# CompVis/ipoke

Measured on AMD Instinct MI355X. Metric: video-frames/sec (second-stage train step), higher is better.
Workload: dtype bf16; 1 GPU; plants_128 second_stage train, 16x3x128x128 clips, z=64, flow 2048 hidden (1.237 B params), per-GPU batch 20; global_batch=20, clip_frames=16, parallelism=dp1, weights=random init of the named architecture (no checkpoints offline)

## Files before the change

### include/ipoke_hip.h

```cpp
#ifndef IPOKE_HIP_H
#define IPOKE_HIP_H

#include <stdint.h>

#ifdef __cplusplus
extern "C" {
#endif

typedef enum {
  IPOKE_OK = 0,
  IPOKE_ERR_INVALID = -1,
  IPOKE_ERR_HIP = -2,
  IPOKE_ERR_STATE = -3
} ipoke_status;

enum { IPOKE_F32 = 0, IPOKE_BF16 = 1 };
enum { IPOKE_ACT_NONE = 0, IPOKE_ACT_ELU = 1, IPOKE_ACT_RELU = 2, IPOKE_ACT_LRELU02 = 3, IPOKE_ACT_TANH = 4,
       IPOKE_ACT_SIGMOID = 5 };

const char* ipoke_last_error(void);
int ipoke_version(void);
int ipoke_dtype_size(int dtype);

typedef struct {
// ... 22 lines not shown
  int32_t c_scatter;
  int64_t c_sn, c_sh, c_sw, c_row0;
  const float* row_scale;
  int32_t rs_images, rs_stride;
  int32_t w_kmajor;
  int64_t c_sd;
  void* acc_scratch;
  int64_t acc_scratch_bytes;
} ipoke_conv_desc;

int ipoke_conv_forward(const ipoke_conv_desc* d, int dtype, void* stream);
int64_t ipoke_conv_acc_scratch_bytes(int M, int Nout, int splitk);
int ipoke_conv_acc_scratch_init(void* scratch, void* stream);

int ipoke_conv3x3_skinny_splitk(int M, int Kc, int dtype);

typedef struct {
  float* params; float* m; float* v; float* vmax; void* operand;
  float lr, beta1, beta2, eps, weight_decay, grad_scale;
  int32_t step;
  int32_t keep_grad;
} ipoke_wgrad_adam;

typedef struct {
  int32_t NB, Di, Hi, Wi, Do, Ho, Wo, kd, kh, kw, sd, sh, sw, pd, ph, pw, transposed;
  const void* A; int32_t a_f32; int64_t a_sn, a_sd, a_sh, a_sw, a_sc; int32_t a_coff, Kc_real, Kc;
  const void* dY; int32_t ldy; int32_t y_coff; int32_t Nout;
  float* dW; int64_t w_sn, w_sc, w_st;
  int32_t accumulate;
  int32_t splitm;
// ... 377 lines not shown
```

### include/ipoke_hip_dev.h

```cpp
#ifndef IPOKE_HIP_DEV_H
#define IPOKE_HIP_DEV_H

#include "ipoke_hip.h"

#ifdef __cplusplus
extern "C" {
#endif

int ipoke_conv_forward_repeat(const ipoke_conv_desc* d, int dtype, int n, void* stream);
int ipoke_set_dispatch_override(const char* name, int value);
enum { IPOKE_KERNEL_NONE = 0, IPOKE_KERNEL_IGEMM = 1, IPOKE_KERNEL_S8 = 2, IPOKE_KERNEL_HALO = 3, IPOKE_KERNEL_HALO16 = 4, IPOKE_KERNEL_C64 = 5, IPOKE_KERNEL_K8 = 6 };
int ipoke_last_conv_kernel(void);
enum { IPOKE_WGRAD_KERNEL_NONE = 0, IPOKE_WGRAD_KERNEL_TN = 1, IPOKE_WGRAD_KERNEL_TN_GLDS = 2, IPOKE_WGRAD_KERNEL_TN_NARROW = 3,
       IPOKE_WGRAD_KERNEL_LAT8 = 4, IPOKE_WGRAD_KERNEL_HALO = 5 };
int ipoke_last_wgrad_kernel(void);

int ipoke_spin_delay(int us, void* stream);

#define IPOKE_TAG_NT_SQUARE 1
#define IPOKE_TAG_TN_SQUARE 2
#define IPOKE_TAG_UNIT_FWD 3
#define IPOKE_TAG_UNIT_BWD 4
#define IPOKE_TAG_UNIT_INV 5
#define IPOKE_TAG_NN_SQUARE 6
#define IPOKE_TAG_CONV_BASE 16
#define IPOKE_TAG_WGRAD 32
int ipoke_timing_start(void);
int ipoke_timing_start_all(void);
int ipoke_timing_stop(const int* tags, int ntags, int* counts, double* mean_us);
int ipoke_timing_stop_ex(const int* tags, int ntags, int* counts, double* total_us, double* flops, double* bytes);

int ipoke_desc_sizes(int32_t* out, int n);

int ipoke_flow_test_inject_timeout(ipoke_flow* f, int which, void* stream);

int ipoke_gru_set_fused(int mode);

#ifdef __cplusplus
}
#endif
#endif
```

### ipoke_amd/_lib.py

```python
import ctypes
import os
from ctypes import CFUNCTYPE, POINTER, Structure, c_char_p, c_float, c_int, c_int32, c_int64, c_uint32, c_void_p

_HERE = os.path.dirname(os.path.abspath(__file__))
LIB_PATH = os.environ.get("IPOKE_LIB_PATH") or os.path.join(_HERE, "libipoke_hip.so")

F32, BF16 = 0, 1
ACT_NONE, ACT_ELU, ACT_RELU, ACT_LRELU02, ACT_TANH, ACT_SIGMOID = range(6)

DTYPES = {"f32": F32, "fp32": F32, "float32": F32, "bf16": BF16, "bfloat16": BF16}


class ConvDesc(Structure):
    _fields_ = [(n, c_int32) for n in ("NB", "Di", "Hi", "Wi", "Do", "Ho", "Wo", "kd", "kh", "kw", "sd", "sh", "sw",
                                       "pd", "ph", "pw", "transposed")] + [
        ("A", c_void_p), ("a_f32", c_int32),
        ("a_sn", c_int64), ("a_sd", c_int64), ("a_sh", c_int64), ("a_sw", c_int64), ("a_sc", c_int64),
        ("a_coff", c_int32), ("Kc_real", c_int32), ("Kc", c_int32),
        ("W", c_void_p), ("ldw", c_int32), ("Nout", c_int32),
        ("bias", c_void_p), ("act", c_int32), ("dact", c_void_p), ("ld_dact", c_int32), ("dact_act", c_int32),
        ("C", c_void_p), ("c_f32", c_int32), ("c_accumulate", c_int32), ("ldc", c_int64),
        ("c_coff", c_int32), ("c_cstride", c_int32), ("splitk", c_int32),
        ("c_scatter", c_int32), ("c_sn", c_int64), ("c_sh", c_int64), ("c_sw", c_int64), ("c_row0", c_int64),
        ("row_scale", c_void_p), ("rs_images", c_int32), ("rs_stride", c_int32), ("w_kmajor", c_int32), ("c_sd", c_int64),
# ... 104 lines not shown
    "ipoke_conv_forward": (c_int, [POINTER(ConvDesc), c_int, _P]),
    "ipoke_conv_forward_repeat": (c_int, [POINTER(ConvDesc), c_int, c_int, _P]),
    "ipoke_set_dispatch_override": (c_int, [c_char_p, c_int]),
    "ipoke_last_conv_kernel": (c_int, []),
    "ipoke_last_wgrad_kernel": (c_int, []),
    "ipoke_gru_set_fused": (c_int, [c_int]),
    "ipoke_gru_workspace_bytes": (c_int64, [POINTER(GruDesc), c_int]),
    "ipoke_gru_unroll_forward": (c_int, [POINTER(GruDesc), _P, c_int, _P, c_int, POINTER(c_void_p), _P, _P, c_int, c_int, _P]),
    "ipoke_gru_unroll_backward": (c_int, [POINTER(GruDesc), _P, c_int, _P, POINTER(c_void_p), _P, _P, c_int, _P]),
    "ipoke_rowscale_bwd_workspace_floats": (c_int64, [c_int64, c_int, c_int64]),
    "ipoke_rowscale_bwd": (c_int, [POINTER(RowScaleBwdDesc), c_int, _P]),
    "ipoke_spectral_bwd_frames": (c_int, [_P, c_int, c_int, c_int, c_int, _P, _P, c_int64, _P, c_int64, _P, c_int, _P]),
    "ipoke_sum_frames": (c_int, [_P, _P, c_int, c_int64, c_int, _P]),
    "ipoke_desc_sizes": (c_int, [POINTER(c_int32), c_int]),
    "ipoke_conv3x3_skinny_splitk": (c_int, [c_int, c_int, c_int]),
    "ipoke_conv3x3_coupling_splitk": (c_int, [c_int, c_int, c_int]),
    "ipoke_conv3x3_coupling_xchg_bytes": (c_int64, []),
    "ipoke_conv3x3_coupling_xchg_init": (c_int, [_P, _P]),
    "ipoke_conv3x3_coupling": (c_int, [POINTER(ConvDesc), POINTER(AffineDesc), POINTER(CouplingEpi), c_int, c_int, _P]),
    "ipoke_conv_wgrad": (c_int, [POINTER(WgradDesc), c_int, _P]),
    "ipoke_wgrad_batch_entry_size": (c_int, []),
    "ipoke_conv_wgrad_batched": (c_int, [POINTER(WgradDesc), _P, c_int, _P, _P, _P, c_int, _P]),
    "ipoke_reduce_entry_size": (c_int, []),
    "ipoke_reduce_rows_multi": (c_int, [_P, _P, _P, c_int, c_int, _P]),
    "ipoke_nchw_to_state": (c_int, [_P, _P, c_int, c_int, c_int, c_int, _P]),
    "ipoke_state_to_nchw": (c_int, [_P, _P, c_int, c_int, c_int, c_int, _P]),
    "ipoke_extract_cols": (c_int, [_P, c_int, c_int, c_int, c_int, _P, c_int, c_int64, c_int, _P]),
    "ipoke_copy_cols": (c_int, [_P, c_int, _P, c_int, c_int, c_int64, c_int, _P]),
    "ipoke_cond_prepare": (c_int, [_P, _P, c_int, c_int, c_int, c_int, c_int, _P]),
    "ipoke_actnorm_fwd": (c_int, [_P, _P, c_int, c_int, c_int, c_int, _P, _P, _P, _P]),
# ... 118 lines not shown
    "ipoke_poke_simulate": (c_int, [_P, c_int, c_int, c_int, c_int, c_int, c_int, c_int, _P, _P, _P, _P, _P, _P, _P, _P]),
    "ipoke_poke_stamp": (c_int, [_P, _P, _P, c_int, c_int, c_int, c_int, c_int, c_int, _P, _P]),
    "ipoke_poke_randomize_workspace_bytes": (c_int64, [c_int, c_int, c_int, c_int]),
    "ipoke_poke_randomize": (c_int, [_P, _P, _P, c_int, c_int, c_int, c_int, c_int, c_int, _P, _P, _P, _P, _P]),
    "ipoke_timing_start": (c_int, []),
    "ipoke_timing_start_all": (c_int, []),
    "ipoke_timing_stop": (c_int, [POINTER(c_int), c_int, POINTER(c_int), POINTER(ctypes.c_double)]),
    "ipoke_timing_stop_ex": (c_int, [POINTER(c_int), c_int, POINTER(c_int), POINTER(ctypes.c_double), POINTER(ctypes.c_double),
                                     POINTER(ctypes.c_double)]),
    "ipoke_flow_create": (c_int, [POINTER(FlowConfig), POINTER(c_void_p)]),
    "ipoke_flow_destroy": (None, [_P]),
    "ipoke_flow_piece_ranges": (c_int, [_P, c_int, POINTER(c_int64), c_int]),
    "ipoke_flow_handoff_timeouts": (c_int, [_P, POINTER(c_uint32)]),
    "ipoke_flow_side_stream": (c_void_p, [_P]),
    "ipoke_flow_test_inject_timeout": (c_int, [_P, c_int, _P]),
    "ipoke_conv_wgrad_splitm": (c_int, [_P, c_int, c_int]),
    "ipoke_conv_acc_scratch_bytes": (c_int64, [c_int, c_int, c_int]),
    "ipoke_conv_acc_scratch_init": (c_int, [_P, _P]),
    "ipoke_flow_param_count": (c_int64, [_P]),
    "ipoke_flow_index_count": (c_int64, [_P]),
    "ipoke_flow_tensor_count": (c_int32, [_P]),
    "ipoke_flow_op_count": (c_int32, [_P]),
    "ipoke_flow_tensor_info": (c_int, [_P, c_int, c_char_p, c_int, POINTER(c_int64), POINTER(c_int32), POINTER(c_int64),
                                       POINTER(c_int32)]),
    "ipoke_flow_shadow_bytes": (c_int64, [_P]),
    "ipoke_flow_set_graph": (c_int, [_P, c_int]),
    "ipoke_flow_float_buffer_count": (c_int64, [_P]),
    "ipoke_flow_set_float_buffers": (c_int, [_P, _P]),
    "ipoke_lu_job_size": (c_int, []),
    "ipoke_lu_prepare": (c_int, [_P, _P, _P, _P, c_int, _P]),
# ... 70 lines not shown
```

### ipoke_amd/csrc/flow_engine.hip

```cpp
#include <functional>
#include <memory>
#include <vector>
#include <string>
#include <cstring>

#include "common.h"

namespace ipoke {

enum OpType { OP_ACTNORM = 0, OP_MCF = 1, OP_NICE = 2, OP_LU = 3 };
enum TensorKind { TK_PARAM = 0, TK_IDX_FWD = 1, TK_IDX_BWD = 2, TK_FLAG = 3, TK_FBUF = 4 };

struct TensorInfo {
  std::string name;
  int64_t offset;
  std::vector<int64_t> shape;
  int kind;
};

struct Op {
  int type = 0;
  int C = 0;
  int c0 = 0, Cn = 0;
  int64_t p_ls = -1, p_bias = -1, idx_fwd = -1, idx_bwd = -1;
// ... 61 lines not shown
  hipStream_t side = nullptr;
  std::vector<hipStream_t> lanes;
  int n_lanes = 1;
  std::vector<hipEvent_t> events; size_t ev_next = 0;
  bool use_side = true;
  struct GraphEntry { std::vector<uintptr_t> key; hipGraph_t graph = nullptr; hipGraphExec_t exec = nullptr; int state = 0; uint64_t used = 0; };
  std::vector<GraphEntry> graphs; hipStream_t cap = nullptr; bool use_graph = false; uint64_t tick = 0;
  struct Unit { int64_t p_lo, p_hi; int wj_lo, wj_hi, row_lo, row_hi; int kind; int op_lo, op_hi; int64_t p2_lo = -1, p2_hi = -1; };
  std::vector<Unit> units;
  std::vector<int> red_first;
  int last_fwd_B = 0; bool have_saved = false;
  int P = 64;
  int unit_split = 1; void* d_xchg = nullptr;
  bool coupling_fuse = false; void* d_cxchg = nullptr;
  void* d_acc = nullptr; int64_t acc_bytes = 0;
  unsigned* h_tmo = nullptr; hipEvent_t pass_ev = nullptr; hipStream_t pass_stream = nullptr; bool pass_recorded = false, pass_unchecked = false;
  int64_t xchg_bytes = 0;
  bool mcf_xop = false;
  bool c2_straight = false;
  struct NativeAdam { bool on = false; float* m = nullptr; float* v = nullptr; float* vmax = nullptr; float lr = 0, beta1 = 0, beta2 = 0, eps = 0, wd = 0,
                      grad_scale = 1; int step = 0, max_blocks = 0; } nadam;
};

namespace {

int64_t align_up(int64_t v, int64_t a) { return (v + a - 1) / a * a; }

struct Builder {
  ipoke_flow& f;
  explicit Builder(ipoke_flow& fl) : f(fl) {}
// ... 1008 lines not shown
  hipLaunchKernelGGL(handoff_poll_kernel, dim3(1), dim3(64), 0, s, reinterpret_cast<const unsigned*>(f->d_xchg),
                     reinterpret_cast<const unsigned*>(f->d_cxchg), f->h_tmo);
  IPK_LAUNCH_CHECK();
  IPK_HIP(hipEventRecord(f->pass_ev, s));
  f->pass_stream = s; f->pass_recorded = true; f->pass_unchecked = true;
  return IPOKE_OK;
}
__global__ void handoff_inject_kernel(unsigned* word) { if (threadIdx.x == 0) atomicAdd(word, 1u); }
extern "C" int ipoke_flow_test_inject_timeout(ipoke_flow* f, int which, void* stream) {
  IPK_REQUIRE(f && (which == 0 || which == 1), "bad arguments");
  int rc = ensure_device(f); if (rc) return rc;
  unsigned* w = reinterpret_cast<unsigned*>(which == 0 ? f->d_xchg : f->d_cxchg);
  IPK_REQUIRE(w != nullptr, "this flow has no such scratch (unit_split = 1 / coupling fusion off)");
  hipLaunchKernelGGL(handoff_inject_kernel, dim3(1), dim3(64), 0, reinterpret_cast<hipStream_t>(stream), w);
  IPK_LAUNCH_CHECK();
  return IPOKE_OK;
}
extern "C" int ipoke_flow_handoff_timeouts(ipoke_flow* f, uint32_t* out) {
  IPK_REQUIRE(f && out, "null argument");
  out[0] = out[1] = 0;
  IPK_HIP(hipDeviceSynchronize());
  if (f->d_xchg) IPK_HIP(hipMemcpy(&out[0], f->d_xchg, sizeof(uint32_t), hipMemcpyDeviceToHost));
  if (f->d_cxchg) IPK_HIP(hipMemcpy(&out[1], f->d_cxchg, sizeof(uint32_t), hipMemcpyDeviceToHost));
  return IPOKE_OK;
}

static int run_forward(ipoke_flow* f, const float* params, const int32_t* perm, const void* shadow, const float* x_nchw,
                       const float* cond_nchw, int B, float* out_nchw, float* logdet, void* workspace, int save, int init,
                       float* params_mut, hipStream_t stream_h) {
  void* stream = reinterpret_cast<void*>(stream_h);
// ... 548 lines not shown
          rc = ipoke_actnorm_affine_bwd(an.c0, an.Cn, an.p_ls >= 0 ? params + an.p_ls : nullptr, an.idx_fwd >= 0 ? perm + an.idx_fwd : nullptr,
                                        gin, l.state(i + 1), an.p_ls >= 0 ? l.dbp(i + 1, 2 * an.Cn) : nullptr, op.cout, op.t_off, op.t_stride,
                                        f->P, l.ld, xin, l.rowsf(op.ws_c, op.cout), l.dld(), gout, dprm, op.Kc3, l.dbp(i, 2 * op.cout), l.B,
                                        l.dtype, l.stream());
        } else {
          rc = ipoke_affine_bwd(op.cout, op.t_off, op.t_stride, f->P, l.ld, gin, xin, l.rowsf(op.ws_c, op.cout), l.dld(), gout, dprm,
                                op.Kc3, l.dbp(i, 2 * op.cout), l.B, l.dtype, l.stream());
        }
        if (rc) return rc;
        ipoke_conv_desc d;
        set_conv8(d, l.B, 3, 1); d.transposed = 1;
        set_a_dense(d, dprm, op.Kc3, op.Kc3);
        d.W = l.sh(op.sh_c3t); d.ldw = 9 * op.Kc3; d.Nout = hid; d.dact = h2; d.ld_dact = op.hidK; d.dact_act = IPOKE_ACT_ELU;
        d.C = dp2; d.ldc = hid;
        rc = ipoke_conv_forward(&d, l.dtype, l.stream()); if (rc) return rc;
        set_conv8(d, l.B, 1, 0);
        set_a_dense(d, dp2, hid, hid);
        if (f->c2_straight) { d.W = l.sh(op.sh_c2); d.w_kmajor = 1; }
        else d.W = l.sh(op.sh_c2t);
        d.ldw = hid; d.Nout = hid; d.dact = h1; d.ld_dact = hid; d.dact_act = IPOKE_ACT_ELU;
        d.C = dp1; d.ldc = hid;
        rc = ipoke_conv_forward(&d, l.dtype, l.stream()); if (rc) return rc;
        set_conv8(d, l.B, 3, 1); d.transposed = 1;
        set_a_dense(d, dp1, hid, hid);
        d.W = l.sh(op.sh_c1t); d.ldw = 9 * hid; d.Nout = op.cin; d.C = gout; d.c_f32 = 1; d.c_accumulate = 1; d.ldc = l.ld;
        d.c_coff = op.z_off; d.c_cstride = op.z_stride; d.splitk = nice_splitk(l);
        if (lanes.size() == 1 && op.cin <= 64) { d.acc_scratch = f->d_acc; d.acc_scratch_bytes = f->acc_bytes; }
        rc = ipoke_conv_forward(&d, l.dtype, l.stream()); if (rc) return rc;
      }
    }
    if (op.type == OP_MCF) {
      if (pend_lo >= 0 && (f->ops[pend_op].C != op.C || pend_hi - pend_lo + 1 >= 256)) { rc = flush_mcf(); if (rc) return rc; }
      if (pend_lo < 0) { pend_hi = op.mcf_idx; pend_op = i; }
      pend_lo = op.mcf_idx;
    } else if (op.type == OP_NICE) {
      pend_nice.push_back(i);
      if (pending_an == i + 1) pending_an = -1;
    }
    if (!(op.type == OP_NICE && op.pair_unit >= 0)) cur ^= 1;
    if (i == f->units[pieces[pk].first].op_lo) {
      rc = finish_piece(pieces[pk].first, pieces[pk].second, pk); if (rc) return rc;
      ++pk;
// ... 39 lines not shown
```

### ipoke_amd/csrc/gemm.hip

```cpp
#include "common.h"
#include <atomic>
#include <cstring>
#include <mutex>
#include <type_traits>

namespace ipoke {

static constexpr int kPitch = 144;

struct GeomDev {
  int M;
  int lDo, lHo, lWo;
  int Do, Ho, Wo, pow2, S;
  int Di, Hi, Wi;
  int khw, kw, taps;
  int sd, sh, sw, pd, ph, pw;
  int lsd, lsh, lsw;
  int transposed;
};

struct NtParams {
  GeomDev g;
  const void* A; int a_f32; long a_sn, a_sd, a_sh, a_sw, a_sc; int a_coff, Kc_real, Kc;
  const void* W; int ldw; int Nout; int Ktot;
// ... 2281 lines not shown
            pack_t o;
#pragma unroll
            for (int e = 0; e < 4; ++e) o[e] = ET<T>::from_f32(v4[e]);
            *reinterpret_cast<pack_t*>(Cp) = o;
          } else {
            for (int e = 0; e < 4; ++e)
              if (n + e < p.n_pad) Cp[e] = ET<T>::from_f32(v4[e]);
          }
        }
      }
    }
  }
  wait_vmcnt<0>();
}

static std::atomic<int> g_c64_mode{1}, g_halo16_mode{1};

static bool c64_applicable(const NtParams& p) {
  const int mode = g_c64_mode.load(std::memory_order_relaxed);
  const GeomDev& g = p.g;
  if (!mode) return false;
  const int kh = g.kw > 0 ? g.khw / g.kw : 0;
  const int lo_y = g.transposed ? g.ph - (kh - 1) : -g.ph, hi_y = g.transposed ? g.ph : kh - 1 - g.ph;
  const int lo_x = g.transposed ? g.pw - (g.kw - 1) : -g.pw, hi_x = g.transposed ? g.pw : g.kw - 1 - g.pw;
  const int nch = p.Kc / 64;
  const bool can = !p.a_f32 && !p.dact && g.taps == g.khw && kh >= 1 && g.khw == kh * g.kw && g.Di == 1 && g.Do == 1 && g.pd == 0 &&
                   g.Hi == g.Ho && g.Wi == g.Wo && g.Ho % 16 == 0 && g.Wo % 16 == 0 && g.sd == 1 && g.sh == 1 && g.sw == 1 &&
                   lo_y >= -1 && hi_y <= 1 && lo_x >= -1 && hi_x <= 1 && (!g.transposed || (kh == 3 && g.kw == 3)) &&
                   (p.Kc == 64 || p.Kc == 128) && p.Kc_real == p.Kc && g.khw * nch <= 9 && (g.khw > 1 || p.c_scatter) && p.Nout <= 64 && (p.a_coff & 7) == 0 &&
                   p.ldw >= p.Ktot && (p.ldw & 7) == 0 && p.splitk == 1 && !p.c_acc && ((p.a_sn | p.a_sh | p.a_sw) & 7) == 0 && p.n_pad <= 64 &&
                   (reinterpret_cast<uintptr_t>(p.W) & 15) == 0;
// ... 590 lines not shown
  IPK_LAUNCH_CHECK();
  return IPOKE_OK;
}
static int dispatch_nn(NtParams& p, hipStream_t s) {
  const GeomDev& g = p.g;
  IPK_REQUIRE(g.taps == 1 && !g.transposed && g.sd == 1 && g.sh == 1 && g.sw == 1 && g.pd == 0 && g.ph == 0 && g.pw == 0 && !p.a_f32 &&
              p.Kc == p.Kc_real && p.Kc % 64 == 0 && (p.a_coff & 7) == 0 && (p.a_sw & 7) == 0 && (p.ldw & 7) == 0 && p.ldw >= p.Nout &&
              p.splitk == 1 && !p.c_scatter && p.a_sh == (long)g.Wi * p.a_sw && p.a_sn == (long)g.Hi * g.Wi * p.a_sw &&
              (long)g.M * p.a_sw + p.Kc < (1L << 31) && (long)p.Ktot * p.ldw < (1L << 31),
              "K-major weights: 1x1 kernel over dense bf16 channels-last rows, K a multiple of 64");
  const int M = g.M;
  const long tn128 = ceil_div(p.Nout, 128);
  int best = 128; long best_cost = ((long)ceil_div(M, 128) * tn128 + 255) / 256 * 128;
  if (M % 160 == 0) { const long c = ((long)(M / 160) * tn128 + 255) / 256 * 160; if (c <= best_cost) { best = 160; best_cost = c; } }
  if (M % 80 == 0) { const long c = ((long)(M / 80) * tn128 + 255) / 256 * 80; if (c < best_cost) { best = 80; best_cost = c; } }
  if (best == 80) return launch_nn_glds<1, 4, 5, 3, 2>(p, s);
  if (best == 160) return launch_nn_glds<2, 4, 5, 3, 1>(p, s);
  return launch_nn_glds<2, 4, 4, 3, 1>(p, s);
}

template <int NSTAGE, int RM, bool NARROW = false, bool ADAM = false>
__global__ __launch_bounds__(512) void igemm_tn_glds_kernel(const TnParams pin) {
  if (IPK_KERNARG_PREFETCH) kernarg_prefetch<(int)sizeof(TnParams)>();
  typedef bf16_t T;
  TnParams p = pin;
  if (pin.batch) {
    const TnBatchEntry e = pin.batch[blockIdx.z + pin.z0];
    p.A = pin.a_base + e.a_off; p.dY = pin.y_base + e.y_off; p.dW = pin.w_base + e.w_off;
    p.g.khw = e.kh * e.kw; p.g.kw = e.kw; p.g.taps = e.kh * e.kw; p.g.ph = e.ph; p.g.pw = e.pw;
    if constexpr (ADAM) { p.ad_p += e.w_off; p.ad_m += e.w_off; p.ad_v += e.w_off; p.ad_vmax += e.w_off; p.ad_sh += e.sh_off; }
  }
  typedef typename ET<T>::frag frag_t;
  typedef __attribute__((address_space(3))) void lds_void;
// ... 783 lines not shown
  hipLaunchKernelGGL(kern, grid, dim3(256), lds, s, p);
  IPK_LAUNCH_CHECK();
  return IPOKE_OK;
}

}

using namespace ipoke;

#ifdef IPOKE_GEMM_STAMPS
extern "C" void ipoke_gemm_set_stamps(long long* base) { g_gemm_stamps = base; }
#endif

extern "C" int ipoke_set_dispatch_override(const char* name, int value) {
  IPK_REQUIRE(name != nullptr && value <= 2, "bad arguments");
  std::atomic<int>* slot = !strcmp(name, "c64") ? &g_c64_mode : (!strcmp(name, "halo16") ? &g_halo16_mode : nullptr);
  IPK_REQUIRE(slot != nullptr, "unknown dispatch switch (c64 | halo16)");
  slot->store(value < 0 ? 1 : value, std::memory_order_relaxed);
  return IPOKE_OK;
}

extern "C" int ipoke_last_conv_kernel(void) { return g_last_kernel; }
extern "C" int ipoke_last_wgrad_kernel(void) { return g_last_wgrad_kernel; }

namespace ipoke {
static int conv_params(NtParams& p, const ipoke_conv_desc* d, int dtype) {
  IPK_REQUIRE(d != nullptr, "null descriptor");
  IPK_REQUIRE(dtype == IPOKE_F32 || dtype == IPOKE_BF16, "bad dtype");
  const int esz = dtype == IPOKE_BF16 ? 2 : 4, e16 = 16 / esz;
  int rc = make_geom(p.g, d->NB, d->Di, d->Hi, d->Wi, d->Do, d->Ho, d->Wo, d->kd, d->kh, d->kw, d->sd, d->sh, d->sw,
                     d->pd, d->ph, d->pw, d->transposed);
  if (rc) return rc;
// ... 74 lines not shown
            g_last_kernel, d->transposed, d->NB, d->Di, d->Hi, d->Wi, d->Do, d->Ho, d->Wo, d->kd, d->kh, d->kw, d->sd, d->sh, d->sw, d->Kc_real, d->Nout,
            d->a_f32, d->c_f32, p.splitk, d->c_scatter, d->row_scale != nullptr, (long)p.g.M,
            2e-9 * p.g.M * d->Nout * (double)p.g.taps * d->Kc_real / st2, ms * 1e3);
    (void)hipEventDestroy(le0); (void)hipEventDestroy(le1);
  }
  if (ts.slot >= 0) {
    const GeomDev& g = p.g;
    const double stride = g.transposed ? (double)g.sd * g.sh * g.sw : 1.0;
    const double flops = 2.0 * g.M * d->Nout * (double)g.taps * d->Kc_real / stride;
    const double in_rows = (double)d->NB * g.Di * g.Hi * g.Wi;
    const double bytes = in_rows * d->Kc_real * (d->a_f32 ? 4 : esz) + (double)d->Nout * g.taps * d->Kc_real * esz +
                         (double)g.M * d->Nout * (d->c_f32 ? 4 : esz) * (p.splitk > 1 && !d->c_accumulate ? p.splitk : 1);
    ts.annotate(square ? 0 : IPOKE_TAG_CONV_BASE + g_last_kernel, flops, bytes);
  }
  return rc;
}

static int fill_tn(TnParams& p, const ipoke_wgrad_desc* d, int dtype, bool batched) {
  IPK_REQUIRE(d != nullptr, "null descriptor");
  IPK_REQUIRE(dtype == IPOKE_F32 || dtype == IPOKE_BF16, "bad dtype");
  const int esz = dtype == IPOKE_BF16 ? 2 : 4, e16 = 16 / esz;
  int rc = make_geom(p.g, d->NB, d->Di, d->Hi, d->Wi, d->Do, d->Ho, d->Wo, d->kd, d->kh, d->kw, d->sd, d->sh, d->sw,
                     d->pd, d->ph, d->pw, d->transposed);
  if (rc) return rc;
  IPK_REQUIRE(batched || (d->A && d->dY && d->dW), "null tensor");
  IPK_REQUIRE(d->Kc % e16 == 0 && d->Kc >= d->Kc_real && d->Kc_real > 0, "Kc must be a padded multiple of 16 bytes");
  if (!d->a_f32) {
    IPK_REQUIRE(d->a_sc == 1 && d->Kc_real % e16 == 0 && d->a_coff % e16 == 0, "dtype activations: aligned channels-last");
    IPK_REQUIRE(d->a_sn % e16 == 0 && d->a_sd % e16 == 0 && d->a_sh % e16 == 0 && d->a_sw % e16 == 0, "aligned rows");
  }
// ... 95 lines not shown
```

Baseline: 6545 video-frames/sec.

## Fuse 1x1 and 3x3 conv data-gradient pair into one kernel in coupling backward

Adds a fused HIP kernel that computes the 1x1 conv2 data gradient (with the ELU derivative mask) for a 128x128 tile, keeps the result in LDS, and immediately runs the 3x3 transposed conv1 data gradient on the 8x8 latent against streamed weights. The partial sums across hidden tiles are reduced through the split-K accumulation scratch. This removes one kernel launch and the global-memory round trip of the intermediate gradient before conv1 reads it back. The cost is a large 156 KB LDS footprint limiting occupancy, a narrow applicability check, and a bf16-only path.

```diff
diff --git a/include/ipoke_hip.h b/include/ipoke_hip.h
--- a/include/ipoke_hip.h
+++ b/include/ipoke_hip.h
@@ -60,6 +60,9 @@
 int ipoke_conv_acc_scratch_init(void* scratch, void* stream);
 
 int ipoke_conv3x3_skinny_splitk(int M, int Kc, int dtype);
+
+int ipoke_conv_pair_dgrad(const ipoke_conv_desc* conv2, const ipoke_conv_desc* conv1, int dtype, void* stream);
+int ipoke_conv_pair_dgrad_applicable(int M, int hidden, int cin, int dtype, int64_t acc_scratch_bytes);
 
 typedef struct {
   float* params; float* m; float* v; float* vmax; void* operand;
diff --git a/include/ipoke_hip_dev.h b/include/ipoke_hip_dev.h
--- a/include/ipoke_hip_dev.h
+++ b/include/ipoke_hip_dev.h
@@ -34,6 +34,8 @@
 
 int ipoke_flow_test_inject_timeout(ipoke_flow* f, int which, void* stream);
 
+int ipoke_flow_test_split_pair_dgrad(ipoke_flow* f, int on);
+
 int ipoke_gru_set_fused(int mode);
 
 #ifdef __cplusplus
diff --git a/ipoke_amd/_lib.py b/ipoke_amd/_lib.py
--- a/ipoke_amd/_lib.py
+++ b/ipoke_amd/_lib.py
@@ -142,6 +142,8 @@
     "ipoke_sum_frames": (c_int, [_P, _P, c_int, c_int64, c_int, _P]),
     "ipoke_desc_sizes": (c_int, [POINTER(c_int32), c_int]),
     "ipoke_conv3x3_skinny_splitk": (c_int, [c_int, c_int, c_int]),
+    "ipoke_conv_pair_dgrad": (c_int, [POINTER(ConvDesc), POINTER(ConvDesc), c_int, _P]),
+    "ipoke_conv_pair_dgrad_applicable": (c_int, [c_int, c_int, c_int, c_int, c_int64]),
     "ipoke_conv3x3_coupling_splitk": (c_int, [c_int, c_int, c_int]),
     "ipoke_conv3x3_coupling_xchg_bytes": (c_int64, []),
     "ipoke_conv3x3_coupling_xchg_init": (c_int, [_P, _P]),
@@ -290,6 +292,7 @@
     "ipoke_flow_handoff_timeouts": (c_int, [_P, POINTER(c_uint32)]),
     "ipoke_flow_side_stream": (c_void_p, [_P]),
     "ipoke_flow_test_inject_timeout": (c_int, [_P, c_int, _P]),
+    "ipoke_flow_test_split_pair_dgrad": (c_int, [_P, c_int]),
     "ipoke_conv_wgrad_splitm": (c_int, [_P, c_int, c_int]),
     "ipoke_conv_acc_scratch_bytes": (c_int64, [c_int, c_int, c_int]),
     "ipoke_conv_acc_scratch_init": (c_int, [_P, _P]),
diff --git a/ipoke_amd/csrc/flow_engine.hip b/ipoke_amd/csrc/flow_engine.hip
--- a/ipoke_amd/csrc/flow_engine.hip
+++ b/ipoke_amd/csrc/flow_engine.hip
@@ -99,6 +99,7 @@
   int unit_split = 1; void* d_xchg = nullptr;
   bool coupling_fuse = false; void* d_cxchg = nullptr;
   void* d_acc = nullptr; int64_t acc_bytes = 0;
+  bool split_pair_dgrad = false;
   unsigned* h_tmo = nullptr; hipEvent_t pass_ev = nullptr; hipStream_t pass_stream = nullptr; bool pass_recorded = false, pass_unchecked = false;
   int64_t xchg_bytes = 0;
   bool mcf_xop = false;
@@ -1137,6 +1138,12 @@
   IPK_REQUIRE(w != nullptr, "this flow has no such scratch (unit_split = 1 / coupling fusion off)");
   hipLaunchKernelGGL(handoff_inject_kernel, dim3(1), dim3(64), 0, reinterpret_cast<hipStream_t>(stream), w);
   IPK_LAUNCH_CHECK();
+  return IPOKE_OK;
+}
+extern "C" int ipoke_flow_test_split_pair_dgrad(ipoke_flow* f, int on) {
+  IPK_REQUIRE(f != nullptr, "null flow handle");
+  f->split_pair_dgrad = on != 0;
+  drop_graphs(f);
   return IPOKE_OK;
 }
 extern "C" int ipoke_flow_handoff_timeouts(ipoke_flow* f, uint32_t* out) {
@@ -1715,18 +1722,28 @@
         d.W = l.sh(op.sh_c3t); d.ldw = 9 * op.Kc3; d.Nout = hid; d.dact = h2; d.ld_dact = op.hidK; d.dact_act = IPOKE_ACT_ELU;
         d.C = dp2; d.ldc = hid;
         rc = ipoke_conv_forward(&d, l.dtype, l.stream()); if (rc) return rc;
+        ipoke_conv_desc d1;
         set_conv8(d, l.B, 1, 0);
         set_a_dense(d, dp2, hid, hid);
         if (f->c2_straight) { d.W = l.sh(op.sh_c2); d.w_kmajor = 1; }
         else d.W = l.sh(op.sh_c2t);
         d.ldw = hid; d.Nout = hid; d.dact = h1; d.ld_dact = hid; d.dact_act = IPOKE_ACT_ELU;
         d.C = dp1; d.ldc = hid;
+        set_conv8(d1, l.B, 3, 1); d1.transposed = 1;
+        set_a_dense(d1, dp1, hid, hid);
+        d1.W = l.sh(op.sh_c1t); d1.ldw = 9 * hid; d1.Nout = op.cin; d1.C = gout; d1.c_f32 = 1; d1.c_accumulate = 1; d1.ldc = l.ld;
+        d1.c_coff = op.z_off; d1.c_cstride = op.z_stride; d1.splitk = nice_splitk(l);
+        if (lanes.size() == 1 && op.cin <= 64) { d1.acc_scratch = f->d_acc; d1.acc_scratch_bytes = f->acc_bytes; }
+        if (lanes.size() == 1 && f->c2_straight && f->d_acc && !f->cfg.condition_nice &&
+            ipoke_conv_pair_dgrad_applicable((int)l.M, hid, op.cin, l.dtype, f->acc_bytes)) {
+          if (!f->split_pair_dgrad) {
+            rc = ipoke_conv_pair_dgrad(&d, &d1, l.dtype, l.stream()); if (rc) return rc;
+            continue;
+          }
+          d1.splitk = hid / 128;
+        }
         rc = ipoke_conv_forward(&d, l.dtype, l.stream()); if (rc) return rc;
-        set_conv8(d, l.B, 3, 1); d.transposed = 1;
-        set_a_dense(d, dp1, hid, hid);
-        d.W = l.sh(op.sh_c1t); d.ldw = 9 * hid; d.Nout = op.cin; d.C = gout; d.c_f32 = 1; d.c_accumulate = 1; d.ldc = l.ld;
-        d.c_coff = op.z_off; d.c_cstride = op.z_stride; d.splitk = nice_splitk(l);
-        if (lanes.size() == 1 && op.cin <= 64) { d.acc_scratch = f->d_acc; d.acc_scratch_bytes = f->acc_bytes; }
+        d = d1;
         rc = ipoke_conv_forward(&d, l.dtype, l.stream()); if (rc) return rc;
       }
     }
diff --git a/ipoke_amd/csrc/gemm.hip b/ipoke_amd/csrc/gemm.hip
--- a/ipoke_amd/csrc/gemm.hip
+++ b/ipoke_amd/csrc/gemm.hip
@@ -2319,7 +2319,7 @@
   wait_vmcnt<0>();
 }
 
-static std::atomic<int> g_c64_mode{1}, g_halo16_mode{1};
+static std::atomic<int> g_c64_mode{1}, g_halo16_mode{1}, g_nn128_mode{1};
 
 static bool c64_applicable(const NtParams& p) {
   const int mode = g_c64_mode.load(std::memory_order_relaxed);
@@ -2940,9 +2940,340 @@
   int best = 128; long best_cost = ((long)ceil_div(M, 128) * tn128 + 255) / 256 * 128;
   if (M % 160 == 0) { const long c = ((long)(M / 160) * tn128 + 255) / 256 * 160; if (c <= best_cost) { best = 160; best_cost = c; } }
   if (M % 80 == 0) { const long c = ((long)(M / 80) * tn128 + 255) / 256 * 80; if (c < best_cost) { best = 80; best_cost = c; } }
+  if (g_nn128_mode.load(std::memory_order_relaxed) == 2) best = 128;
   if (best == 80) return launch_nn_glds<1, 4, 5, 3, 2>(p, s);
   if (best == 160) return launch_nn_glds<2, 4, 5, 3, 1>(p, s);
   return launch_nn_glds<2, 4, 4, 3, 1>(p, s);
+}
+
+struct PairEpi {
+  const void* W1; int ldw1, cin, transposed;
+  float* C2; long ldc2; int c_coff2, c_cstride2;
+  unsigned* acc_cnt; float* acc_part;
+};
+static constexpr int kPairImg = 128 * (128 * 4 + 16), kPairZrow = kPairImg + 2 * 128 * 128, kPairRing = 100 * 1024,
+                     kPairDummy = kPairRing + 12 * 32 * 128;
+static constexpr size_t kLdsPair = kPairDummy + 8 * 1024;
+static_assert(kPairZrow + 256 <= kPairRing && 3 * (128 * 128 + 64 * 256) <= kPairRing, "LDS regions of igemm_nn_pair_kernel overlap");
+
+__global__ __launch_bounds__(512) __attribute__((amdgpu_waves_per_eu(2, 2))) void igemm_nn_pair_kernel(const NtParams p, const PairEpi e) {
+  if (IPK_KERNARG_PREFETCH) kernarg_prefetch<(int)(sizeof(NtParams) + sizeof(PairEpi)) < 512 ? (int)(sizeof(NtParams) + sizeof(PairEpi)) : 512>();
+  typedef bf16_t T;
+  typedef typename ET<T>::frag frag_t;
+  typedef typename Pack4<T>::type pack_t;
+  typedef __attribute__((address_space(3))) void lds_void;
+  typedef const __attribute__((address_space(1))) void glb_void;
+  constexpr int WM = 2, WN = 4, MREP = 4, NREP = 2, NSTAGE = 3, NTHR = 512, NWAVE = 8, BM = 128, BN = 128;
+  constexpr int A_IT = BM * 8 / NTHR, B_IT = 1024 / NTHR, L = A_IT + B_IT;
+  constexpr int SUB = BM * 128 + 64 * 256;
+  constexpr int EP = BN * 4 + 16;
+  constexpr int R = 12, WSLOT = 32 * 128, WJ = 2, ABUF = BM * 128;
+  constexpr int NKB = 18, NROUNDS = 5;
+  constexpr unsigned kInvalid = 0xffffffffu;
+  extern __shared__ __attribute__((aligned(16))) unsigned char smem[];
+  unsigned char* img = smem + kPairImg;
+  unsigned char* zrow = smem + kPairZrow;
+  unsigned char* ring = smem + kPairRing;
+  unsigned char* dummy = smem + kPairDummy;
+  if (p.prio == 1) __builtin_amdgcn_s_setprio(1); else if (p.prio == 2) __builtin_amdgcn_s_setprio(2); else if (p.prio == 3) __builtin_amdgcn_s_setprio(3);
+
+  const int tid = threadIdx.x, lane = tid & 63, wave = tid >> 6;
+  const int wm = wave / WN, wn = wave % WN;
+  const GeomDev& g = p.g;
+  int tm, tn;
+  {
+    const int bid = blockIdx.x;
+    if (p.xa > 0) {
+      const int xcd = bid & 7, q = bid >> 3;
+      const FDiv fxa(p.xa), fxb(p.xb);
+      const int sub_m = fxa.div(p.tiles_m), sub_n = fxb.div(p.tiles_n);
+      const FDiv fsm(sub_m);
+      tm = fxa.mod(xcd) * sub_m + fsm.mod(q);
+      tn = fxa.div(xcd) * sub_n + fsm.div(q);
+    } else {
+      const FDiv ftm(p.tiles_m);
+      tm = ftm.mod(bid); tn = ftm.div(bid);
+    }
+  }
+  const int m0 = tm * BM, n0 = tn * BN;
+  const int hid = p.Nout;
+  const T* zero = reinterpret_cast<const T*>(g_zero_chunk);
+  if (tid < 16) reinterpret_cast<f32x4*>(zrow)[tid] = f32x4{0.f, 0.f, 0.f, 0.f};
+
+  const T* W1 = reinterpret_cast<const T*>(e.W1);
+  unsigned w_src[WJ];
+#pragma unroll
+  for (int j = 0; j < WJ; ++j) {
+    const int n = 8 * WJ * (wave >> 2) + 8 * j + (lane >> 3), pos = lane & 7;
+    w_src[j] = n < e.cin ? (unsigned)((long)n * e.ldw1 + n0 + ((pos ^ ((n >> 1) & 7)) * 8)) : kInvalid;
+  }
+  int wi_g = wave & 3, wi_c = 0, wi_t = wave & 3;
+  auto issue_w = [&]() {
+    const bool in = wi_g < NKB;
+#pragma unroll
+    for (int j = 0; j < WJ; ++j) {
+      const bool real = in && w_src[j] != kInvalid;
+      const T* src = real ? W1 + w_src[j] + (long)wi_t * hid + wi_c * 64 : zero;
+      unsigned char* dst = in ? ring + (wi_g % R) * WSLOT + (WJ * (wave >> 2) + j) * 1024 : dummy + wave * 1024;
+      __builtin_amdgcn_global_load_lds((glb_void*)src, (lds_void*)dst, 16, 0, 0);
+    }
+    wi_g += 4; wi_t += 4;
+    if (wi_t >= 9) { wi_t -= 9; ++wi_c; }
+  };
+  issue_w(); issue_w();
+
+  const int nkb = (p.Ktot + 63) >> 6;
+  unsigned a_off[A_IT];
+#pragma unroll
+  for (int i = 0; i < A_IT; ++i) {
+    const int ch = tid + NTHR * i, row = ch >> 3, pos = ch & 7;
+    a_off[i] = (m0 + row < g.M) ? (unsigned)((long)(m0 + row) * p.a_sw + p.a_coff + ((pos ^ ((row >> 1) & 7)) * 8)) : kInvalid;
+  }
+  unsigned b_off[B_IT]; int b_row[B_IT];
+#pragma unroll
+  for (int i = 0; i < B_IT; ++i) {
+    const int row = 4 * (wave + NWAVE * i) + (lane >> 4), col = n0 + (((lane & 15) ^ tn_swz(row)) * 8);
+    b_row[i] = row;
+    b_off[i] = col < p.Nout ? (unsigned)((long)row * p.ldw + col) : kInvalid;
+  }
+  const T* Abase = reinterpret_cast<const T*>(p.A);
+  const T* Wbase = reinterpret_cast<const T*>(p.W);
+  int kb_issue = 0;
+  auto issue_slot = [&](int slot) {
+    unsigned char* sa = smem + slot * SUB;
+    const bool real = kb_issue < nkb;
+#pragma unroll
+    for (int i = 0; i < A_IT; ++i) {
+      const T* src = (real && a_off[i] != kInvalid) ? Abase + a_off[i] : zero;
+      unsigned char* dst = real ? sa + (wave * 64 + NTHR * i) * 16 : dummy + wave * 1024;
+      __builtin_amdgcn_global_load_lds((glb_void*)src, (lds_void*)dst, 16, 0, 0);
+      if (a_off[i] != kInvalid) a_off[i] += 64;
+    }
+#pragma unroll
+    for (int i = 0; i < B_IT; ++i) {
+      const T* src = (real && b_off[i] != kInvalid && kb_issue * 64 + b_row[i] < p.Ktot) ? Wbase + b_off[i] : zero;
+      unsigned char* dst = real ? sa + BM * 128 + (wave + NWAVE * i) * 1024 : dummy + wave * 1024;
+      __builtin_amdgcn_global_load_lds((glb_void*)src, (lds_void*)dst, 16, 0, 0);
+      if (b_off[i] != kInvalid) b_off[i] += (unsigned)(64 * p.ldw);
+    }
+    ++kb_issue;
+  };
+  f32x4 acc[MREP][NREP];
+#pragma unroll
+  for (int i = 0; i < MREP; ++i)
+#pragma unroll
+    for (int j = 0; j < NREP; ++j) acc[i][j] = f32x4{0.f, 0.f, 0.f, 0.f};
+  {
+    int a_rd[MREP][2];
+#pragma unroll
+    for (int s2 = 0; s2 < 2; ++s2) {
+      const int q = s2 * 4 + (lane >> 4);
+#pragma unroll
+      for (int i = 0; i < MREP; ++i) {
+        const int row = wm * MREP * 16 + i * 16 + (lane & 15);
+        a_rd[i][s2] = row * 128 + ((q ^ ((row >> 1) & 7)) * 16);
+      }
+    }
+    const int i16 = lane & 15, grp = lane >> 4;
+    const int rrow = 8 * grp + (i16 >> 2);
+    const int hsw = tn_swz(rrow);
+    const unsigned lds0 = (unsigned)(unsigned long)(__attribute__((address_space(3))) unsigned char*)smem;
+    unsigned b_rd[NREP];
+#pragma unroll
+    for (int j = 0; j < NREP; ++j) {
+      const int col = (wn * NREP + j) * 16 + 4 * (i16 & 3);
+      b_rd[j] = lds0 + (unsigned)(BM * 128 + rrow * 256 + (((col >> 3) ^ hsw) * 16) + ((col >> 2) & 1) * 8);
+    }
+    auto read_b = [&](frag_t (&fb)[NREP], unsigned sb, int kstep) {
+#pragma unroll
+      for (int j = 0; j < NREP; ++j) {
+        const unsigned a = b_rd[j] + sb + (unsigned)(kstep * 32 * 256);
+        const tn_tr4_t lo = tn_ds_tr<0>(a), hi = tn_ds_tr<4 * 256>(a);
+#pragma unroll
+        for (int q = 0; q < 4; ++q) { fb[j][q] = lo[q]; fb[j][4 + q] = hi[q]; }
+      }
+    };
+    auto wait_b = [&](frag_t (&fb)[NREP]) { asm volatile("s_waitcnt lgkmcnt(0)" : "+v"(fb[0]), "+v"(fb[1])::"memory"); };
+#pragma unroll
+    for (int s2 = 0; s2 < NSTAGE - 1; ++s2) issue_slot(s2);
+    int slot = 0;
+    for (int kb = 0; kb < nkb; ++kb) {
+      wait_vmcnt<(NSTAGE - 2) * L>();
+      __builtin_amdgcn_s_barrier();
+      issue_slot((slot + NSTAGE - 1) % NSTAGE);
+      const unsigned char* base = smem + slot * SUB;
+      const unsigned sb = (unsigned)(slot * SUB);
+      slot = (slot + 1) % NSTAGE;
+      frag_t fa[2][MREP], fb[2][NREP];
+      read_b(fb[0], sb, 0);
+#pragma unroll
+      for (int i = 0; i < MREP; ++i) fa[0][i] = *reinterpret_cast<const frag_t*>(base + a_rd[i][0]);
+      wait_b(fb[0]);
+      read_b(fb[1], sb, 1);
+#pragma unroll
+      for (int i = 0; i < MREP; ++i) fa[1][i] = *reinterpret_cast<const frag_t*>(base + a_rd[i][1]);
+#pragma unroll
+      for (int i = 0; i < MREP; ++i)
+#pragma unroll
+        for (int j = 0; j < NREP; ++j) GEMM_MMA(fa[0][i], fb[0][j], acc[i][j]);
+      wait_b(fb[1]);
+#pragma unroll
+      for (int i = 0; i < MREP; ++i)
+#pragma unroll
+        for (int j = 0; j < NREP; ++j) GEMM_MMA(fa[1][i], fb[1][j], acc[i][j]);
+    }
+  }
+  wait_vmcnt<0>();
+
+  constexpr int G4F = BN / 4, ITER = BM * G4F / NTHR, RSTEP = NTHR / G4F;
+  const int c4 = tid % G4F, r0 = tid / G4F;
+  const bool mask = p.dact != nullptr;
+  pack_t dy[ITER], o[ITER];
+#pragma unroll
+  for (int k = 0; k < ITER; ++k) dy[k] = pack_t{};
+  if (mask) {
+#pragma unroll
+    for (int k = 0; k < ITER; ++k) {
+      const int m = min(m0 + r0 + k * RSTEP, g.M - 1);
+      dy[k] = *reinterpret_cast<const pack_t*>(reinterpret_cast<const T*>(p.dact) + (long)m * p.ld_dact + n0 + 4 * c4);
+    }
+  }
+  auto lds_barrier = [] { asm volatile("s_waitcnt lgkmcnt(0)\n\ts_barrier" ::: "memory"); };
+  lds_barrier();
+  {
+    unsigned char* base = smem + (wm * MREP * 16 + (lane & 15)) * EP + (wn * NREP * 16 + (lane >> 4) * 4) * 4;
+#pragma unroll
+    for (int i = 0; i < MREP; ++i)
+#pragma unroll
+      for (int j = 0; j < NREP; ++j) *reinterpret_cast<f32x4*>(base + i * 16 * EP + j * 64) = acc[i][j];
+  }
+  __syncthreads();
+  {
+    const unsigned char* sp = smem + r0 * EP + c4 * 16;
+    const int pos = (c4 & 15) >> 1;
+#pragma unroll
+    for (int k = 0; k < ITER; ++k) {
+      const int row = r0 + k * RSTEP;
+      const f32x4 v = *reinterpret_cast<const f32x4*>(sp + k * RSTEP * EP);
+#pragma unroll
+      for (int r = 0; r < 4; ++r) {
+        float x = v[r];
+        const float y = ET<T>::to_f32(dy[k][r]);
+        x *= (mask && y <= 0.f) ? y + 1.f : 1.f;
+        o[k][r] = ET<T>::from_f32(m0 + row < g.M ? x : 0.f);
+      }
+      *reinterpret_cast<pack_t*>(img + (c4 >> 4) * ABUF + row * 128 + ((pos ^ ((row >> 1) & 7)) * 16) + (c4 & 1) * 8) = o[k];
+    }
+  }
+
+  constexpr int CREP = 2;
+  const int mh = wave & 1, kq = wave >> 1;
+  const int sgn = e.transposed ? -1 : 1;
+  unsigned vmask[MREP];
+#pragma unroll
+  for (int i = 0; i < MREP; ++i) {
+    const int r = i * 16 + (lane & 15);
+    const int y = (r >> 3) & 7, x = r & 7;
+    unsigned vm = 0;
+#pragma unroll
+    for (int t = 0; t < 9; ++t) {
+      const int yy = y + sgn * (t / 3 - 1), xx = x + sgn * (t % 3 - 1);
+      if ((unsigned)yy < 8u && (unsigned)xx < 8u) vm |= 1u << t;
+    }
+    vmask[i] = vm;
+  }
+  const int qlo = lane >> 4;
+  int w_rd[CREP];
+#pragma unroll
+  for (int j = 0; j < CREP; ++j) {
+    const int n = j * 16 + (lane & 15);
+    w_rd[j] = n * 128 + ((qlo ^ ((n >> 1) & 7)) * 16);
+  }
+  f32x4 acc2[MREP][CREP];
+#pragma unroll
+  for (int i = 0; i < MREP; ++i)
+#pragma unroll
+    for (int j = 0; j < CREP; ++j) acc2[i][j] = f32x4{0.f, 0.f, 0.f, 0.f};
+  int gk = kq, ci = 0, t = kq;
+  for (int r = 0; r < NROUNDS; ++r) {
+    wait_vmcnt<WJ>();
+    lds_barrier();
+    issue_w();
+    if (gk < NKB) {
+      const unsigned char* ab = img + ci * ABUF + mh * 64 * 128;
+      const unsigned char* wb = ring + (gk % R) * WSLOT;
+      const int th = t / 3, tw = t - 3 * th;
+      const int shift = sgn * ((th - 1) * 8 + (tw - 1));
+      const unsigned char* arow[MREP]; int aswz[MREP];
+#pragma unroll
+      for (int i = 0; i < MREP; ++i) {
+        const bool ok = (vmask[i] >> t) & 1u;
+        const int sr = i * 16 + (lane & 15) + shift;
+        arow[i] = ok ? ab + sr * 128 : zrow;
+        aswz[i] = ok ? (sr >> 1) & 7 : 0;
+      }
+      frag_t fa[2][MREP], fb[2][CREP];
+#pragma unroll
+      for (int hs = 0; hs < 2; ++hs) {
+#pragma unroll
+        for (int i = 0; i < MREP; ++i) fa[hs][i] = *reinterpret_cast<const frag_t*>(arow[i] + (((hs * 4 + qlo) ^ aswz[i]) * 16));
+#pragma unroll
+        for (int j = 0; j < CREP; ++j) fb[hs][j] = *reinterpret_cast<const frag_t*>(wb + (w_rd[j] ^ (hs * 64)));
+      }
+#pragma unroll
+      for (int hs = 0; hs < 2; ++hs)
+#pragma unroll
+        for (int i = 0; i < MREP; ++i)
+#pragma unroll
+          for (int j = 0; j < CREP; ++j) GEMM_MMA(fa[hs][i], fb[hs][j], acc2[i][j]);
+      constexpr int NF = MREP + CREP, NM = MREP * CREP, PER = NM / NF;
+      __builtin_amdgcn_sched_group_barrier(0x100, NF, 0);
+#pragma unroll
+      for (int f = 0; f < NF; ++f) {
+        __builtin_amdgcn_sched_group_barrier(0x008, PER, 0);
+        __builtin_amdgcn_sched_group_barrier(0x100, 1, 0);
+      }
+      __builtin_amdgcn_sched_group_barrier(0x008, 2 * NM - NF * PER, 0);
+    }
+    gk += 4; t += 4;
+    if (t >= 9) { t -= 9; ++ci; }
+  }
+  wait_vmcnt<0>();
+  if (c4 * 4 + n0 < p.Nout) {
+    T* Cp = reinterpret_cast<T*>(p.C) + (long)(m0 + r0) * p.ldc + p.c_coff + n0 + 4 * c4;
+#pragma unroll
+    for (int k = 0; k < ITER; ++k)
+      if (m0 + r0 + k * RSTEP < g.M) *reinterpret_cast<pack_t*>(Cp + (long)k * RSTEP * p.ldc) = o[k];
+  }
+  constexpr int EP2 = 16 * CREP * 4 + 16;
+  {
+    unsigned char* st = smem + (mh * MREP * 16 + (lane & 15)) * EP2 + (lane >> 4) * 16;
+    lds_barrier();
+#pragma unroll
+    for (int round = 0; round < 2; ++round) {
+      const int give_lo = round == 0 ? 2 : 1, take_hi = round == 0 ? 2 : 1;
+      if (kq >= give_lo && kq < 2 * give_lo) {
+        unsigned char* d = st + (kq - give_lo) * BM * EP2;
+#pragma unroll
+        for (int i = 0; i < MREP; ++i)
+#pragma unroll
+          for (int j = 0; j < CREP; ++j) *reinterpret_cast<f32x4*>(d + i * 16 * EP2 + j * 64) = acc2[i][j];
+      }
+      lds_barrier();
+      if (kq < take_hi) {
+        const unsigned char* d = st + kq * BM * EP2;
+#pragma unroll
+        for (int i = 0; i < MREP; ++i)
+#pragma unroll
+          for (int j = 0; j < CREP; ++j) acc2[i][j] += *reinterpret_cast<const f32x4*>(d + i * 16 * EP2 + j * 64);
+      }
+      if (round == 0) lds_barrier();
+    }
+  }
+  NtParams q = p;
+  q.splitk = p.tiles_n; q.tiles_n = 1; q.c_acc = 1; q.c_f32 = 1; q.acc_cnt = e.acc_cnt; q.acc_part = e.acc_part;
+  q.C = e.C2; q.ldc = e.ldc2; q.c_coff = e.c_coff2; q.c_cstride = e.c_cstride2; q.Nout = e.cin;
+  nt_epilogue<T, 2, 1, MREP, CREP, NTHR, true>(q, acc2, smem, m0, 0, mh, 0, tn, kq == 0);
 }
 
 template <int NSTAGE, int RM, bool NARROW = false, bool ADAM = false>
@@ -3756,8 +4087,8 @@
 
 extern "C" int ipoke_set_dispatch_override(const char* name, int value) {
   IPK_REQUIRE(name != nullptr && value <= 2, "bad arguments");
-  std::atomic<int>* slot = !strcmp(name, "c64") ? &g_c64_mode : (!strcmp(name, "halo16") ? &g_halo16_mode : nullptr);
-  IPK_REQUIRE(slot != nullptr, "unknown dispatch switch (c64 | halo16)");
+  std::atomic<int>* slot = !strcmp(name, "c64") ? &g_c64_mode : (!strcmp(name, "halo16") ? &g_halo16_mode : (!strcmp(name, "nn128") ? &g_nn128_mode : nullptr));
+  IPK_REQUIRE(slot != nullptr, "unknown dispatch switch (c64 | halo16 | nn128)");
   slot->store(value < 0 ? 1 : value, std::memory_order_relaxed);
   return IPOKE_OK;
 }
@@ -3862,6 +4193,66 @@
     ts.annotate(square ? 0 : IPOKE_TAG_CONV_BASE + g_last_kernel, flops, bytes);
   }
   return rc;
+}
+
+extern "C" int ipoke_conv_pair_dgrad_applicable(int M, int hidden, int cin, int dtype, int64_t acc_scratch_bytes) {
+  if (dtype != IPOKE_BF16 || M < 64 || M % 64 != 0 || hidden < 256 || hidden % 128 != 0 || cin < 1 || cin > 32) return 0;
+  const long tiles = (long)ceil_div(M, 128) * (hidden / 128);
+  if (tiles > 256) return 0;
+  return acc_scratch_bytes >= kAccCounterBytes + tiles * 128 * 32 * 4 ? 1 : 0;
+}
+
+extern "C" int ipoke_conv_pair_dgrad(const ipoke_conv_desc* conv2, const ipoke_conv_desc* conv1, int dtype, void* stream) {
+  IPK_REQUIRE(conv2 != nullptr && conv1 != nullptr, "null descriptor");
+  IPK_REQUIRE(dtype == IPOKE_BF16, "the fused data gradients are bf16 only");
+  NtParams p, p1;
+  int rc = conv_params(p, conv2, dtype); if (rc) return rc;
+  rc = conv_params(p1, conv1, dtype); if (rc) return rc;
+  const GeomDev& g = p.g; const GeomDev& g1 = p1.g;
+  IPK_REQUIRE(conv2->w_kmajor && g.taps == 1 && !g.transposed && g.sd == 1 && g.sh == 1 && g.sw == 1 && g.pd == 0 && g.ph == 0 && g.pw == 0 &&
+              !p.a_f32 && p.Kc == p.Kc_real && p.Kc % 64 == 0 && (p.a_coff & 7) == 0 && (p.a_sw & 7) == 0 && (p.ldw & 7) == 0 &&
+              p.ldw >= p.Nout && p.splitk == 1 && !p.c_scatter && p.a_sh == (long)g.Wi * p.a_sw && p.a_sn == (long)g.Hi * g.Wi * p.a_sw &&
+              (long)g.M * p.a_sw + p.Kc < (1L << 31) && (long)p.Ktot * p.ldw < (1L << 31),
+              "conv2: K-major weights, 1x1 kernel over dense bf16 channels-last rows, K a multiple of 64");
+  IPK_REQUIRE(!p.bias && p.act == IPOKE_ACT_NONE && !p.c_f32 && !p.row_scale && ((p.ldc | p.c_coff) & 3) == 0 && p.ldc >= p.c_coff + p.Nout &&
+              (!p.dact || ((p.ld_dact & 3) == 0 && p.dact_act == IPOKE_ACT_ELU && p.ld_dact >= p.Nout)) &&
+              (long)g.M * p.ldc < (1L << 31) && (long)g.M * p.ld_dact < (1L << 31),
+              "conv2: dense dtype output, no bias / activation, an ELU derivative mask at most");
+  IPK_REQUIRE(!p1.c_scatter && !p1.a_f32 && g1.taps == 9 && g1.khw == 9 && g1.kw == 3 && g1.Di == 1 && g1.Hi == 8 && g1.Wi == 8 &&
+              g1.lDo == 0 && g1.lHo == 3 && g1.lWo == 3 && g1.sd == 1 && g1.sh == 1 && g1.sw == 1 && g1.pd == 0 && g1.ph == 1 && g1.pw == 1 &&
+              g1.M == g.M && p1.Kc == p.Nout && p1.Kc_real == p1.Kc && p1.ldw >= p1.Ktot && (long)p1.Nout * p1.ldw < (1L << 31),
+              "conv1: 3x3 kernel, padding 1, on the 8x8 latent over conv2's output channels");
+  IPK_REQUIRE(p1.A == p.C && p1.a_coff == p.c_coff && p1.a_sw == p.ldc && p1.a_sh == 8 * p.ldc && p1.a_sn == 64 * p.ldc,
+              "conv1 reads conv2's output (same pointer, column offset and row stride)");
+  IPK_REQUIRE(p1.c_f32 && p1.c_acc && !p1.bias && p1.act == IPOKE_ACT_NONE && !p1.dact && !p1.row_scale,
+              "conv1 accumulates raw fp32 sums");
+  IPK_REQUIRE(conv1->acc_scratch != nullptr && ((uintptr_t)conv1->acc_scratch & 15) == 0,
+              "conv1 needs the accumulation scratch (ipoke_conv_acc_scratch_bytes / _init), 16-byte aligned");
+  IPK_REQUIRE(ipoke_conv_pair_dgrad_applicable(g.M, p.Nout, p1.Nout, dtype, conv1->acc_scratch_bytes),
+              "shape not taken by the fused launch (ipoke_conv_pair_dgrad_applicable)");
+  IPK_REQUIRE(kLdsPair <= device_max_lds(), "the fused launch needs 156 KB of LDS per workgroup");
+  hipStream_t s = reinterpret_cast<hipStream_t>(stream);
+  p.prio = 2;
+  p.w_kmajor = 1;
+  g_last_kernel = IPOKE_KERNEL_IGEMM;
+  PairEpi e;
+  e.W1 = p1.W; e.ldw1 = p1.ldw; e.cin = p1.Nout; e.transposed = g1.transposed;
+  e.C2 = reinterpret_cast<float*>(p1.C); e.ldc2 = p1.ldc; e.c_coff2 = p1.c_coff; e.c_cstride2 = p1.c_cstride;
+  e.acc_cnt = reinterpret_cast<unsigned*>(conv1->acc_scratch);
+  e.acc_part = reinterpret_cast<float*>(reinterpret_cast<unsigned char*>(conv1->acc_scratch) + kAccCounterBytes);
+  p.tiles_m = ceil_div(g.M, 128); p.tiles_n = p.Nout / 128;
+  p.splitk = 1; p.kb_per_split = ceil_div(p.Ktot, 64);
+  pick_xcd_map(p);
+  const bool square = p.Nout == p.Ktot && p.Nout >= 1024;
+  TimedScope ts(square ? IPOKE_TAG_NN_SQUARE : IPOKE_TAG_CONV_BASE, s);
+  auto kern = igemm_nn_pair_kernel;
+  IPK_SET_LDS_ONCE(kern, kLdsPair);
+  hipLaunchKernelGGL(kern, dim3((unsigned)((long)p.tiles_m * p.tiles_n)), dim3(512), kLdsPair, s, p, e);
+  IPK_LAUNCH_CHECK();
+  if (ts.slot >= 0)
+    ts.annotate(square ? 0 : IPOKE_TAG_CONV_BASE + IPOKE_KERNEL_IGEMM, 2.0 * g.M * p.Nout * ((double)p.Kc + 9.0 * p1.Nout),
+                2.0 * ((double)g.M * p.Kc + (double)p.Nout * p.Kc + (double)g.M * p.Nout + 9.0 * p1.Nout * p.Nout) + 4.0 * g.M * p1.Nout);
+  return IPOKE_OK;
 }
 
 static int fill_tn(TnParams& p, const ipoke_wgrad_desc* d, int dtype, bool batched) {
```

New measurement: 6669 video-frames/sec (median of 6 runs). 1.02x the previous value.
